# xiaochuanle/hifimeth

Measured on AMD Instinct MI355X. Metric: cytosine sites/sec (CpG+CHG+CHH), higher is better.
Workload: dtype f16x3+f32acc

## Files before the change

hifimeth_amd/csrc/hm_engine.cpp:

```cpp
#include <hip/hip_runtime.h>

#include <algorithm>
#include <atomic>
#include <cmath>
#include <condition_variable>
#include <cstdio>
#include <cstring>
#include <memory>
#include <mutex>
#include <string>
#include <thread>
#include <vector>

#include "../../include/hifimeth_hip.h"
#include "hm_device.h"
#include "hm_host.h"
#include "hm_kernels.h"
#include "hm_weights.h"

using namespace hm;

namespace {

thread_local std::string g_create_error;

enum Kind { K_PREP, K_SCAN, K_EMIT, K_PACK, K_WINDOW, K_FRONT, K_TAIL, K_TRUNK, K_EDGE, K_TAILG };

struct TimedSpan {
    int kind, ctx;
    int64_t off, cap;
    Event a, b;
};

struct DeviceModel {
    bool loaded = false;
    int k1 = 0;
    DevBuf params;
    CtxWeights w{};
};

}

struct hm_batch {
    hm_engine* e = nullptr;
    int id = 0;
    enum State { FREE, STAGING, QUEUED } state = FREE;
    bool uploaded = false, ran = false, have_totals = false, have_calls = false;
    Stream s_io;
    Event ev_in, ev_comp, ev_out;

    PinnedArr<uint8_t> slab;
    PinnedArr<ReadDesc> reads;
    PinnedArr<Chunk> chunks;
    PinnedArr<RInfo> rinfo;
    PinnedArr<TrunkTile> tiles;
    PinnedArr<int32_t> tcost;
    struct Group {
        int chunk_lo, chunk_hi, tile_lo, tile_hi;
        int64_t bases, rows;
        int cost_lo;
    };
    std::vector<Group> groups;
    int64_t total_bases = 0;

    DevBuf d_raw, d_reads, d_chunks, d_rinfo, d_tiles, d_tcost, d_bases, d_kin, d_sctx, d_counts, d_offs, d_totals, d_err;
    DevBuf d_usites, d_utag, d_csites, d_opos, d_logits, d_p, d_ml, d_calls;
    Pinned<int32_t> h_totals;
    Pinned<int32_t> h_err;
    PinnedArr<hm_call_t> h_calls;
    int32_t totals[TOT_COUNT] = {};

    std::vector<TimedSpan> spans;

    ~hm_batch() {
        if (s_io) (void)hipStreamSynchronize(s_io);
    }
};

namespace {

struct GroupBufs {
    DevBuf d_map[3], d_e4, d_edge4, d_e4row, d_rowlist;
    DevBuf d_x6;
    DevBuf d_mark, d_ccnt, d_order, d_okey;
    DevBuf d_odst;
    DevBuf d_x8;
    DevBuf d_dump;
    int64_t bytes() const {
        const DevBuf* all[] = {&d_map[0], &d_map[1], &d_map[2], &d_e4, &d_edge4, &d_e4row, &d_rowlist, &d_x6, &d_mark, &d_ccnt, &d_order, &d_okey, &d_odst, &d_x8, &d_dump};
        static_assert(sizeof(GroupBufs) == sizeof all / sizeof *all * sizeof(DevBuf), "a member of GroupBufs is missing from bytes()");
        int64_t sum = 0;
        for (const DevBuf* d : all) sum += (int64_t)d->cap;
        return sum;
    }
};

}

struct hm_engine {
    int device = 0;
    int num_cu = 256;
    int ctx_mask = 7;
    int min_read_size = 1000;
    int64_t sub_batch = 65536;
    int front_waves = 8;
    int precision = 1;
    int conv3_w16 = 0;
    int max_slots = 3;
    int trunk = 2;
    int trunk_impl = 3;
    int edge_impl = 1;
    int tail_impl = 3;
    int64_t tail_slice = int64_t(1) << 21;
    int trunk_mask_auto = -1;
    int64_t group_bases = 0;
    std::atomic<int64_t> group_bases_eff{0};
    bool stamps_on = false;
    std::vector<unsigned long long> stamp_sum;
    bool timing = false;
    std::string err;

    std::mutex mu;
    std::mutex order_mu;
    std::condition_variable cv;
    hm_timing_t acc{};
    int64_t x6_sites = 0;

    Stream stream;
    std::vector<Event> pool;
    DevBuf d_act4, d_win, d_dbg, d_stamps, d_zeros;
    GroupBufs grp;
    DeviceModel model[3];
    std::vector<std::unique_ptr<hm_batch>> slots;

    ~hm_engine() {
        (void)hipSetDevice(device);
        if (stream) (void)hipStreamSynchronize(stream);
    }
};

namespace {

constexpr int64_t GROUP_BYTES_PER_BASE = (3 * 2 * 512 + 2 * 384 + 768 + 4 + 8 + 2 * 4 + 8 + 4 + TAIL_STRIP_HANDOVER_BYTES) * 5 / 4;

int64_t effective_group_bases(hm_engine* e) {
    if (e->group_bases > 0) return e->group_bases;
    if (const int64_t have = e->group_bases_eff.load(std::memory_order_relaxed)) return have;
    size_t free_b = 0, total_b = 0;
    int64_t gb = int64_t(2) << 20;
    int prev = -1;
    (void)hipGetDevice(&prev);
    if (hipSetDevice(e->device) == hipSuccess && hipMemGetInfo(&free_b, &total_b) == hipSuccess && free_b > 0) {
        gb = (int64_t)(free_b / 4) / GROUP_BYTES_PER_BASE;
        gb = std::min<int64_t>(gb, int64_t(16) << 20);
        gb = std::max<int64_t>(gb >> 20 << 20, int64_t(1) << 20);
    }
    if (prev >= 0 && prev != e->device) (void)hipSetDevice(prev);
    int64_t none = 0;
    if (!e->group_bases_eff.compare_exchange_strong(none, gb, std::memory_order_relaxed)) gb = none;
    return gb;
}

constexpr int TILE_COST = 8, TILE_COST_CONST = 1;
void add_read_tiles(hm_engine* e, hm_batch* b, int ridx, int l_qseq) {
    if (b->groups.empty() || b->groups.back().rows >= effective_group_bases(e)) {
        b->groups.push_back(hm_batch::Group{(int)b->chunks.n, (int)b->chunks.n, (int)b->tiles.n, (int)b->tiles.n, 0, 0, (int)b->tcost.n});
        b->tcost.push_back(0);
    }
    hm_batch::Group& g = b->groups.back();
    const int ntile = (l_qseq + 2 * TR_PAD + TR_OWN - 1) / TR_OWN;
    b->rinfo.push_back(RInfo{b->total_bases, l_qseq, (int32_t)g.rows});
    for (int t = 0; t < ntile; ++t) {
        const int u0 = -TR_PAD + t * TR_OWN;
        b->tiles.push_back(TrunkTile{ridx, u0});
        b->tcost.push_back(b->tcost.p[b->tcost.n - 1] + (t == 0 ? 2 * TILE_COST_CONST : u0 >= l_qseq ? TILE_COST_CONST : TILE_COST));
    }
    for (int st = 0; st < l_qseq; st += CHUNK) b->chunks.push_back(Chunk{ridx, st});
    g.rows += (int64_t)ntile * TR_OWN + TR_SLACK;
    if (2 * g.rows >= (int64_t(1) << 27)) throw HipErr{hipErrorInvalidValue, "a read group's maps exceed 2^27 rows (group_bases too large)"};
    g.bases += l_qseq;
    g.chunk_hi = (int)b->chunks.n;
    g.tile_hi = (int)b->tiles.n;
}

int fail(hm_engine* e, int code, const std::string& msg) {
    if (e) {
        std::lock_guard<std::mutex> lk(e->mu);
        e->err = msg;
    } else {
        g_create_error = msg;
    }
    return code;
}

int fail_hip(hm_engine* e, const HipErr& h) {
    return fail(e, HM_EDEVICE, hip_error_text(h));
}

template <class Body>
auto guarded(hm_engine* e, Body&& body) -> decltype(body()) {
    return hip_guard(e->device, [e](const HipErr& h) { return fail_hip(e, h); }, body);
}

Event get_event(hm_engine* e) {
    Event ev;
    {
        std::lock_guard<std::mutex> lk(e->mu);
        if (!e->pool.empty()) {
            ev = std::move(e->pool.back());
            e->pool.pop_back();
            return ev;
        }
    }
    HIP_TRY(hipEventCreate(&ev.h));
    return ev;
}

struct Span {
    hm_engine* e;
    std::vector<TimedSpan>* sink;
    TimedSpan ts{};
    bool on;
    Span(hm_engine* eng, std::vector<TimedSpan>* out, int kind, int ctx = 0, int64_t off = 0, int64_t cap = 0)
        : e(eng), sink(out), on(eng->timing && out) {
        if (!on) return;
        ts.kind = kind;
        ts.ctx = ctx;
        ts.off = off;
        ts.cap = cap;
        ts.a = get_event(e);
        ts.b = get_event(e);
        HIP_TRY(hipEventRecord(ts.a, e->stream));
    }
    void end() {
        if (!on) return;
        HIP_TRY(hipEventRecord(ts.b, e->stream));
        sink->push_back(std::move(ts));
        on = false;
    }
};

void collect_timing(hm_engine* e, std::vector<TimedSpan>& spans, const int32_t* totals) {
    if (!spans.empty() && totals) {
        std::lock_guard<std::mutex> lk(e->mu);
        for (int c = 0; c < 3; ++c) e->acc.trunk_list_steps[c] += totals[TOT_LIST_STEPS + c];
        for (int c = 0; c < 3; ++c) e->acc.trunk_const_steps[c] += totals[TOT_CONST_STEPS + c];
        e->acc.tail_strip_passes += totals[TOT_STRIP_PASSES];
    }
    for (auto& s : spans) {
        float ms = 0.f;
        HIP_TRY(hipEventElapsedTime(&ms, s.a, s.b));
        std::lock_guard<std::mutex> lk(e->mu);
        hm_timing_t& t = e->acc;
        const int64_t n = totals ? std::clamp<int64_t>((int64_t)totals[s.ctx] - s.off, 0, s.cap) : s.cap;
        switch (s.kind) {
        case K_PREP: t.prep_ms += ms; ++t.prep_launches; break;
        case K_SCAN: t.scan_ms += ms; ++t.scan_launches; break;
        case K_EMIT: t.emit_ms += ms; ++t.emit_launches; break;
        case K_PACK: t.pack_ms += ms; ++t.pack_launches; break;
        case K_WINDOW: t.window_ms += ms; ++t.window_launches; t.window_sites += s.cap; break;
        case K_TRUNK: t.trunk_ms[s.ctx] += ms; ++t.trunk_launches[s.ctx]; t.trunk_positions[s.ctx] += s.cap; break;
        case K_EDGE: t.edge_ms[s.ctx] += ms; ++t.edge_launches[s.ctx]; break;
        case K_TAILG: t.tail_ms[s.ctx] += ms; ++t.tail_launches[s.ctx]; break;
        case K_FRONT:
            if (n > 0) { t.front_ms[s.ctx] += ms; ++t.front_launches[s.ctx]; t.front_sites[s.ctx] += n; }
            else { t.empty_ms += ms; ++t.empty_launches; }
            break;
        default:
            if (n > 0) { t.tail_ms[s.ctx] += ms; ++t.tail_launches[s.ctx]; }
            else { t.empty_ms += ms; ++t.empty_launches; }
            break;
        }
        e->pool.push_back(std::move(s.a));
        e->pool.push_back(std::move(s.b));
    }
    spans.clear();
}

void upload_model(hm_engine* e, int ctx, const HostModel& hmw) {
    DeviceModel& dm = e->model[ctx];
    PackedModel pk = pack_model(hmw);
    dm.params.reserve(pk.blob.size() * sizeof(float));
    HIP_TRY(hipMemcpy(dm.params.p, pk.blob.data(), pk.blob.size() * sizeof(float), hipMemcpyHostToDevice));
    const float* base = dm.params.as<float>();
    for (int i = 0; i < 9; ++i) {
        dm.w.wfrag[i] = base + pk.wfrag_off[i];
        dm.w.bias[i] = base + pk.bias_off[i];
    }
    dm.w.fc2_w = base + pk.fc2_w_off;
    dm.w.fc2_b = base + pk.fc2_b_off;
    dm.w.bn = reinterpret_cast<const BnTables*>(base + pk.bn_off);
    for (int i = 0; i < 9; ++i) dm.w.wfrag_h[i] = reinterpret_cast<const uint16_t*>(base + pk.wfrag_h_off[i]);
    dm.w.bn_h = reinterpret_cast<const BnTablesH*>(base + pk.bn_h_off);
    dm.w.c1f = reinterpret_cast<const uint16_t*>(base + pk.c1f_off);
    dm.w.c1f_bias = base + pk.c1f_bias_off;
    dm.w.c1f_corr = base + pk.c1f_corr_off;
    dm.w.k1 = hmw.k1;
    dm.k1 = hmw.k1;
    dm.loaded = true;
}

size_t align16(size_t x) { return (x + 15) & ~size_t(15); }

void accumulate_stamps(hm_engine* e) {
    const int ns = front_stamp_slots();
    const size_t n = (size_t)e->num_cu * 8 * ns;
    std::vector<unsigned long long> h(n);
    HIP_TRY(hipStreamSynchronize(e->stream));
    HIP_TRY(hipMemcpy(h.data(), e->d_stamps.p, n * sizeof(unsigned long long), hipMemcpyDeviceToHost));
    HIP_TRY(hipMemset(e->d_stamps.p, 0, n * sizeof(unsigned long long)));
    e->stamp_sum.resize((size_t)ns * 8, 0);
    for (size_t i = 0; i < n; ++i) e->stamp_sum[i % ((size_t)ns * 8)] += h[i];
}

void launch_cnn_pair(hm_engine* e, std::vector<TimedSpan>* spans, int ctx, const SiteRange& sr, const hm_batch* b,
                     const float* windows, float* logits, float* p, uint8_t* ml, float* dbg, int dbg_layer) {
    const DeviceModel& dm = e->model[ctx];
    const ReadDesc* reads = b ? b->d_reads.as<ReadDesc>() : nullptr;
    const uint8_t* bases = b ? b->d_bases.as<uint8_t>() : nullptr;
    const uint32_t* kin = b ? b->d_kin.as<uint32_t>() : nullptr;
    {
        Span sp(e, spans, K_FRONT, ctx, sr.off, sr.cap);
        if (e->precision >= 1)
            launch_front_h(e->stream, dm.k1, sr, reads, bases, kin, windows, dm.w, e->d_act4.as<float>(), e->num_cu, dbg,
                           dbg_layer, e->stamps_on ? e->d_stamps.as<unsigned long long>() : nullptr, false);
        else
            launch_front(e->stream, dm.k1, sr, reads, bases, kin, windows, dm.w, e->d_act4.as<float>(), e->num_cu, dbg,
                         dbg_layer, e->front_waves, e->stamps_on ? e->d_stamps.as<unsigned long long>() : nullptr);
        if (e->stamps_on) accumulate_stamps(e);
        sp.end();
    }
    {
        Span sp(e, spans, K_TAIL, ctx, sr.off, sr.cap);
        if (e->precision >= 1)
            launch_tail_h(e->stream, e->d_act4.as<float>(), sr, dm.w, logits, p, ml, e->num_cu, dbg, dbg_layer, 0);
        else
            launch_tail(e->stream, e->d_act4.as<float>(), sr, dm.w, logits, p, ml, e->num_cu, dbg, dbg_layer);
        sp.end();
    }
}

void run_cnn_windows(hm_engine* e, int ctx, const float* windows, int64_t n, float* logits, float* p, uint8_t* ml,
                     float* dbg, int dbg_layer) {
    const int64_t sb = e->sub_batch;
    e->d_act4.reserve((size_t)std::min<int64_t>(std::max<int64_t>(n, 1), sb) * ACT4_FLOATS * sizeof(float));
    std::vector<TimedSpan> spans;
    for (int64_t off = 0; off < n; off += sb) {
        const int m = (int)std::min<int64_t>(sb, n - off);
        const SiteRange sr{nullptr, nullptr, ctx, 0, m};
        launch_cnn_pair(e, e->timing ? &spans : nullptr, ctx, sr, nullptr, windows + (size_t)off * KMER * FEATS,
                        logits + 2 * off, p + off, ml + off, dbg, dbg_layer);
    }
    HIP_TRY(hipGetLastError());
    HIP_TRY(hipStreamSynchronize(e->stream));
    collect_timing(e, spans, nullptr);
}

hm_batch* new_slot(hm_engine* e, int id) {
    std::unique_ptr<hm_batch> b(new hm_batch());
    b->e = e;
    b->id = id;
    HIP_TRY(hipStreamCreateWithFlags(&b->s_io.h, hipStreamNonBlocking));
    for (Event* ev : {&b->ev_in, &b->ev_comp, &b->ev_out}) HIP_TRY(hipEventCreateWithFlags(&ev->h, hipEventDisableTiming));
    b->h_totals.alloc(TOT_COUNT);
    b->h_err.alloc();
    b->d_totals.reserve(TOT_COUNT * sizeof(int32_t));
    b->d_err.reserve(sizeof(int32_t));
    HIP_TRY(hipMemset(b->d_err.p, 0, sizeof(int32_t)));
    HIP_TRY(hipMemset(b->d_totals.p, 0, TOT_COUNT * sizeof(int32_t)));
    hm_batch* raw = b.get();
    e->slots.push_back(std::move(b));
    return raw;
}

void reset_staging(hm_batch* b) {
    b->slab.n = 0;
    b->reads.n = 0;
    b->chunks.n = 0;
    b->rinfo.n = 0;
    b->tiles.n = 0;
    b->tcost.n = 0;
    b->groups.clear();
    b->total_bases = 0;
    b->uploaded = b->ran = b->have_totals = b->have_calls = false;
    memset(b->totals, 0, sizeof b->totals);
}


int check_read(hm_engine* e, const hm_read_t& r, int64_t tb, const char* who, const char* full) {
    if (r.l_qseq < 0) return fail(e, HM_EINVAL, std::string(who) + ": negative read length");
    if (r.l_qseq < e->min_read_size) return 0;
    if (!r.kin[0] || !r.kin[1] || !r.kin[2] || !r.kin[3]) return 0;
    if (!r.seq4) return fail(e, HM_EINVAL, std::string(who) + ": seq4 is NULL");
    for (int k = 0; k < 4; ++k)
        if (r.width[k] != 1 && r.width[k] != 2) return fail(e, HM_EINVAL, "kinetics element width must be 1 (B:C) or 2 (B:S)");
    if (tb + (int64_t)r.l_qseq + 4 >= (int64_t(1) << 31)) return fail(e, HM_ENOMEM, std::string(who) + ": batch would exceed 2^31 bases; " + full);
    return 1;
}

int64_t padded_bases(int32_t l_qseq) { return ((int64_t)l_qseq + 3) & ~int64_t(3); }

struct SlabCopy {
    const void* src;
    size_t off, bytes;
};

void place_read(hm_batch* b, const hm_read_t& r, SlabCopy* copies) {
    const size_t L = (size_t)r.l_qseq;
    auto place = [&](const void* src, size_t bytes) {
        const int64_t off = (int64_t)b->slab.n;
        *copies++ = SlabCopy{src, (size_t)off, bytes};
        b->slab.n += align16(bytes);
        return off;
    };
    ReadDesc rd{};
    rd.off_seq = place(r.seq4, (L + 1) / 2);
    rd.off_fi = place(r.kin[0], L * r.width[0]);
    rd.off_fp = place(r.kin[1], L * r.width[1]);
    rd.off_ri = place(r.kin[2], L * r.width[2]);
    rd.off_rp = place(r.kin[3], L * r.width[3]);
    rd.base_off = b->total_bases;
    rd.len = r.l_qseq;
    rd.flag = r.flag;
    rd.read_id = r.read_id;
    for (int k = 0; k < 4; ++k) rd.w[k] = r.width[k];
    const int ridx = (int)b->reads.n;
    b->reads.push_back(rd);
    add_read_tiles(b->e, b, ridx, r.l_qseq);
    b->total_bases += padded_bases(r.l_qseq);
}

int stage_read(hm_batch* b, int32_t read_id, int32_t l_qseq, int32_t flag, const uint8_t* seq4, const void* fi, int fi_w,
               const void* fp, int fp_w, const void* ri, int ri_w, const void* rp, int rp_w) {
    auto width = [](int w) { return (uint8_t)std::clamp(w, 0, 255); };
    const hm_read_t r{read_id, l_qseq, flag, {width(fi_w), width(fp_w), width(ri_w), width(rp_w)}, seq4, {fi, fp, ri, rp}};
    const int rc = check_read(b->e, r, b->total_bases, "hm_submit_read", "flush / queue it first");
    if (rc <= 0) return rc;
    return guarded(b->e, [&] {
        const size_t L = (size_t)l_qseq;
        const size_t need = align16((L + 1) / 2) + align16(L * fi_w) + align16(L * fp_w) + align16(L * ri_w) + align16(L * rp_w);
        if (b->slab.n + need > b->slab.cap) b->slab.reserve(std::max<size_t>((b->slab.n + need) * 2, size_t(64) << 20));
        SlabCopy copies[5];
        place_read(b, r, copies);
        for (const SlabCopy& c : copies) memcpy(b->slab.p + c.off, c.src, c.bytes);
        return 1;
    });
}

void enqueue_upload(hm_batch* b) {
    const size_t nr = b->reads.n, nc = b->chunks.n;
    b->d_raw.reserve(std::max<size_t>(b->slab.n, 16));
    b->d_reads.reserve(std::max<size_t>(nr, 1) * sizeof(ReadDesc));
    b->d_chunks.reserve(std::max<size_t>(nc, 1) * sizeof(Chunk));
    const size_t tb = (size_t)std::max<int64_t>(b->total_bases, 4);
    b->d_bases.reserve(tb);
    b->d_sctx.reserve(tb);
    b->d_kin.reserve(tb * sizeof(uint32_t));
    b->d_counts.reserve((nc + 1) * NCNT * sizeof(int32_t));
    b->d_offs.reserve((nc + 1) * NCNT * sizeof(int32_t));
    b->d_usites.reserve(tb * sizeof(USite));
    b->d_utag.reserve(tb);
    b->d_csites.reserve(tb * sizeof(Site));
    b->d_opos.reserve(tb * sizeof(int32_t));
    b->d_logits.reserve(tb * 2 * sizeof(float));
    b->d_p.reserve(tb * sizeof(float));
    b->d_ml.reserve(tb);
    b->d_calls.reserve(tb * sizeof(hm_call_t));
    if (b->slab.n) HIP_TRY(hipMemcpyAsync(b->d_raw.p, b->slab.p, b->slab.n, hipMemcpyHostToDevice, b->s_io));
    if (nr) HIP_TRY(hipMemcpyAsync(b->d_reads.p, b->reads.p, nr * sizeof(ReadDesc), hipMemcpyHostToDevice, b->s_io));
    if (nc) HIP_TRY(hipMemcpyAsync(b->d_chunks.p, b->chunks.p, nc * sizeof(Chunk), hipMemcpyHostToDevice, b->s_io));
    b->d_rinfo.reserve(std::max<size_t>(nr, 1) * sizeof(RInfo));
    b->d_tiles.reserve(std::max<size_t>(b->tiles.n, 1) * sizeof(TrunkTile));
    if (nr) HIP_TRY(hipMemcpyAsync(b->d_rinfo.p, b->rinfo.p, nr * sizeof(RInfo), hipMemcpyHostToDevice, b->s_io));
    if (b->tiles.n) HIP_TRY(hipMemcpyAsync(b->d_tiles.p, b->tiles.p, b->tiles.n * sizeof(TrunkTile), hipMemcpyHostToDevice, b->s_io));
    b->d_tcost.reserve(std::max<size_t>(b->tcost.n, 1) * sizeof(int32_t));
    if (b->tcost.n) HIP_TRY(hipMemcpyAsync(b->d_tcost.p, b->tcost.p, b->tcost.n * sizeof(int32_t), hipMemcpyHostToDevice, b->s_io));
    HIP_TRY(hipEventRecord(b->ev_in, b->s_io));
    b->uploaded = true;
    b->ran = b->have_totals = b->have_calls = false;
}

void run_trunk_path(hm_batch* b, std::vector<TimedSpan>* spans, int ctx_mask) {
    hm_engine* e = b->e;
    int64_t max_rows = 1, max_bases = 1;
    for (const auto& g : b->groups) {
        max_rows = std::max(max_rows, g.rows);
        max_bases = std::max(max_bases, g.bases);
    }
    for (int i = 0; i < 3; ++i) e->grp.d_map[i].reserve((size_t)max_rows * 2 * 256 * sizeof(uint16_t));
    e->grp.d_e4.reserve((size_t)max_rows * 2 * C4_CH * sizeof(float));
    e->grp.d_rowlist.reserve(std::max((size_t)(max_rows / TR_OWN + 1) * 2 * 3 * TR_OWN, trunk3_rowlist_bytes((max_rows / TR_OWN + 1) * 2)));
    e->grp.d_dump.reserve(trunk3_dump_bytes(e->num_cu));
    e->grp.d_edge4.reserve((size_t)max_bases * 2 * C4_CH * sizeof(float));
    e->grp.d_e4row.reserve((size_t)max_bases * sizeof(int32_t));
    if (e->tail_impl == 3 && e->precision >= 1 && (ctx_mask >> CHH & 1)) {
        e->grp.d_mark.reserve(tail_strip_mark_bytes(2 * max_rows));
        e->grp.d_ccnt.reserve(tail_strip_count_bytes(2 * max_rows));
        e->grp.d_order.reserve((size_t)max_bases * sizeof(int32_t));
        e->grp.d_okey.reserve((size_t)max_bases * sizeof(int32_t));
        e->grp.d_odst.reserve((size_t)max_bases * sizeof(int32_t));
        e->grp.d_x8.reserve(tail_strip_handover_bytes(max_bases));
    }
    if (!e->d_zeros.p) {
        e->d_zeros.reserve(1024);
        HIP_TRY(hipMemsetAsync(e->d_zeros.p, 0, 1024, e->stream));
    }
    const bool w16 = false;
    const int32_t* offs = b->d_offs.as<int32_t>();
    for (const auto& g : b->groups) {
        const TrunkMaps maps{{e->grp.d_map[0].as<uint16_t>(), e->grp.d_map[1].as<uint16_t>(), e->grp.d_map[2].as<uint16_t>()},
                             e->grp.d_e4.as<uint16_t>(), g.rows, e->d_zeros.as<uint16_t>(), e->grp.d_rowlist.as<uint8_t>()};
        const int n_tiles = g.tile_hi - g.tile_lo;
        for (int c = 0; c < 3; ++c) {
            if (!(ctx_mask >> c & 1)) continue;
            const DeviceModel& dm = e->model[c];
            const int n_views = c == CHH ? 2 : 1;
            const SiteRange sr{b->d_csites.as<Site>(), b->d_totals.as<int32_t>(), c, 0, (int32_t)std::min<int64_t>(g.bases, INT32_MAX),
                               offs + (size_t)NCNT * g.chunk_lo + c, offs + (size_t)NCNT * g.chunk_hi + c};
            if (e->precision == 0) {
                {
                    Span sp(e, spans, K_TRUNK, c, 0, (int64_t)n_tiles * TR_OWN * n_views);
                    launch_trunk_f32(e->stream, dm.k1, b->d_tiles.as<TrunkTile>() + g.tile_lo, n_tiles, n_views, c, b->d_rinfo.as<RInfo>(),
                                     b->d_bases.as<uint8_t>(), b->d_kin.as<uint32_t>(), b->d_sctx.as<uint8_t>(), dm.w, maps, e->num_cu);
                    sp.end();
                }
                {
                    Span sp(e, spans, K_EDGE, c);
                    launch_edge_f32(e->stream, dm.k1, sr, b->d_rinfo.as<RInfo>(), b->d_bases.as<uint8_t>(), b->d_kin.as<uint32_t>(), dm.w,
                                    maps, e->grp.d_edge4.as<float>(), e->grp.d_e4row.as<int32_t>(), e->num_cu);
                    sp.end();
                }
                Span sp(e, spans, K_TAILG, c);
                launch_tail_gather_f32(e->stream, sr, dm.w, maps, e->grp.d_edge4.as<float>(), e->grp.d_e4row.as<int32_t>(),
                                       b->d_logits.as<float>(), b->d_p.as<float>(), b->d_ml.as<uint8_t>(), e->num_cu);
                sp.end();
                continue;
            }
            {
                Span sp(e, spans, K_TRUNK, c, 0, (int64_t)n_tiles * TR_OWN * n_views);
                if (e->trunk_impl == 3)
                    launch_trunk3(e->stream, dm.k1, b->d_tiles.as<TrunkTile>() + g.tile_lo, n_tiles, n_views, c, b->d_rinfo.as<RInfo>(),
                                  b->d_bases.as<uint8_t>(), b->d_kin.as<uint32_t>(), b->d_sctx.as<uint8_t>(), b->total_bases, dm.w, maps, e->grp.d_dump.as<uint16_t>(),
                                  b->d_totals.as<int32_t>() + TOT_LIST_STEPS, b->d_tcost.as<int32_t>() + g.cost_lo, e->num_cu, e->conv3_w16 != 0);
                else if (e->trunk_impl)
                    launch_trunk2(e->stream, dm.k1, b->d_tiles.as<TrunkTile>() + g.tile_lo, n_tiles, n_views, c, b->d_rinfo.as<RInfo>(),
                                  b->d_bases.as<uint8_t>(), b->d_kin.as<uint32_t>(), b->d_sctx.as<uint8_t>(), dm.w, maps, e->num_cu, w16,
                                  e->trunk_impl == 2);
                else
// ... 689 lines not shown
```

hifimeth_amd/csrc/hm_trunk3.hip:

```cpp
#include "hm_convh.h"
#ifdef HM_TRUNK_STAMP
#include "hm_stamp.h"
namespace hm { __device__ unsigned long long g_trunk3_stamp[8][24]; }
extern "C" int hm_debug_trunk3_stamps(unsigned long long* out, int reset) {
    if (out && hipMemcpyFromSymbol(out, HIP_SYMBOL(hm::g_trunk3_stamp), sizeof(hm::g_trunk3_stamp)) != hipSuccess) return -1;
    if (reset) {
        static unsigned long long z[8][24];
        if (hipMemcpyToSymbol(HIP_SYMBOL(hm::g_trunk3_stamp), z, sizeof(z)) != hipSuccess) return -1;
    }
    return 0;
}
#endif
#include "hm_convs.h"
#include "hm_edge.h"

namespace hm {

namespace {

constexpr int T3_M = TR_OWN;
constexpr int T3_H1 = 4, T3_H2 = 8, T3_H3 = 16;
constexpr int T3_S3 = T3_H3, T3_S2 = T3_S3 + T3_H2, T3_S1 = T3_S2 + T3_H1;
constexpr int T3_AROWS = T3_M + T3_H3, T3_BROWS = T3_M + T3_H2;
constexpr int T3_XROWS = 128;
constexpr int T3_LDS_HALVES = 2 * T3_AROWS * TR_RS + 2 * T3_BROWS * TR_RS + 2 * (T3_H1 + T3_H3) * TR_RS;
constexpr int T3_N4 = 64, T3_RL3 = 3 * TR_OWN, T3_RL = T3_RL3 + T3_N4 + 4;
constexpr int T3_RLW = 3 * 32 + T3_N4 / 4 + 1;
static_assert(T3_M % 16 == 0 && T3_RL % 4 == 0 && T3_RL / 4 <= 256 && T3_XROWS >= T3_M + 12, "tile plan");

struct ListRows4 {
    static constexpr bool DENSE = false;
    static constexpr int M = T3_N4;
    const uint8_t* rows = nullptr;
    template <class C>
    __device__ __forceinline__ int off(int m) const { return (int)rows[m] * C::IRS; }
};
struct EpiE4L {
    half_t* __restrict__ g;
    const uint8_t* rows;
    __device__ __forceinline__ void operator()(int m, int col, const f32x4& acc) const {
        half4 h, l;
        split4(acc, h, l);
        const size_t o = (size_t)rows[m] * (2 * C4_CH) + col;
        *reinterpret_cast<half4*>(g + o) = h;
        *reinterpret_cast<half4*>(g + o + C4_CH) = l;
    }
};

struct EpiTrunk3 {
    half_t* hi;
    half_t* lo;
    __device__ __forceinline__ void operator()(int m, int col, const f32x4& acc) const {
        half4 h, l;
        split4(acc, h, l);
        *reinterpret_cast<half4*>(hi + m * TR_RS + col) = h;
        *reinterpret_cast<half4*>(lo + m * TR_RS + col) = l;
    }
};
struct EpiE43 {
    half_t* __restrict__ g;
    __device__ __forceinline__ void operator()(int m, int col, const f32x4& acc) const {
        half4 h, l;
        split4(acc, h, l);
        *reinterpret_cast<half4*>(g + (size_t)m * (2 * C4_CH) + col) = h;
        *reinterpret_cast<half4*>(g + (size_t)m * (2 * C4_CH) + C4_CH + col) = l;
    }
};
template <int NWV_>
struct CopyRows3 {
    static constexpr int NWV = NWV_, CS = TR_OWN / (2 * NWV_);
    const uint8_t* rows;
    half_t* g;
};

__device__ __forceinline__ void t3_lds_barrier() {
    __builtin_amdgcn_fence(__ATOMIC_RELEASE, "workgroup", "local");
    __builtin_amdgcn_s_barrier();
    __builtin_amdgcn_fence(__ATOMIC_ACQUIRE, "workgroup", "local");
}

template <int NROWS, int NT, int K = 0>
__device__ __forceinline__ void move_rows(half_t* dh, half_t* dl, const half_t* sh, const half_t* sl, int t) {
    constexpr int PER = NROWS * TR_RS / 8, N = 2 * PER;
    if constexpr (K * NT < N) {
        const int c = min(t + K * NT, N - 1), plane = c >= PER, o = (c - plane * PER) * 8;
        const uint4 v = *reinterpret_cast<const uint4*>((plane ? sl : sh) + o);
        move_rows<NROWS, NT, K + 1>(dh, dl, sh, sl, t);
        *reinterpret_cast<uint4*>((plane ? dl : dh) + o) = v;
    }
}

}

constexpr int T3_RPB = 4;
template <int K1>
__global__ __launch_bounds__(64) void rowlist3_kernel(const TrunkTile* __restrict__ tiles, int n_tiles, int n_work, int ctx,
                                                       const RInfo* __restrict__ rinfo, const uint8_t* __restrict__ sctx, int64_t n_bases,
                                                       uint8_t* __restrict__ rowlist) {
    using G = EdgeGeo<K1>;
    const int r = threadIdx.x;
    constexpr int first_new[3] = {T3_H1, T3_H2, T3_H3}, shift[3] = {T3_S1, T3_S2, T3_S3};
    constexpr int W0 = -176, WN = 528;
    __shared__ __attribute__((aligned(4))) uint8_t rec[T3_RPB][T3_RL];
    __shared__ __attribute__((aligned(4))) uint8_t sf[T3_RPB][WN];
    static_assert(-G::R1 - 2 + T3_S1 >= W0 && -G::R2 - 4 + T3_S2 >= W0 && -G::R3 - 8 + T3_S3 >= W0 && T3_S1 + TR_OWN - 1 - G::LEFT < W0 + WN &&
                  215 - 16 * 23 >= W0 && TR_OWN - 1 + 215 - 16 < W0 + WN, "the window covers every lookup");
    int kind[T3_RPB];
    TrunkTile tl[T3_RPB];
    RInfo ri[T3_RPB];
    bool warm[T3_RPB];
    int view[T3_RPB];
#pragma unroll
    for (int k = 0; k < T3_RPB; ++k) {
        const int blk = (int)blockIdx.x * T3_RPB + k;
        kind[k] = blk > 2 * n_work ? 0 : blk == 2 * n_work ? 2 : 1;
        warm[k] = blk >= n_work;
        const int w = min(warm[k] ? blk - n_work : blk, n_work - 1);
        view[k] = w >= n_tiles;
        tl[k] = tiles[view[k] ? w - n_tiles : w];
    }
    bool any = false;
#pragma unroll
    for (int k = 0; k < T3_RPB; ++k) {
        if (kind[k] == 1 && warm[k] && tl[k].u0 != -TR_PAD) kind[k] = 0;
        any |= kind[k] != 0;
    }
    if (!any) return;
#pragma unroll
    for (int k = 0; k < T3_RPB; ++k) ri[k] = rinfo[tl[k].read_idx];
    constexpr int NQ = (WN / 4 + 63) / 64;
    static_assert(WN % 4 == 0 && (-W0) % 4 == 0 && TR_PAD % 4 == 0 && TR_OWN % 4 == 0, "windows start on multiples of 4");
    uint32_t sw[T3_RPB][NQ];
#pragma unroll
    for (int k = 0; k < T3_RPB; ++k) {
        const int L = ri[k].len, u = tl[k].u0 - (warm[k] ? TR_OWN : 0);
#pragma unroll
        for (int q = 0; q < NQ; ++q) {
            const int y0 = u + W0 + 4 * (r + 64 * q);
            const int64_t a = view[k] ? ri[k].base_off + (L - 1 - y0 - 3) : ri[k].base_off + y0;
            if (a >= 0 && a + 4 <= n_bases) {
                uint32_t v;
                __builtin_memcpy(&v, sctx + a, 4);
                sw[k][q] = view[k] ? __builtin_bswap32(v) : v;
            } else {
                uint32_t v = 0;
#pragma unroll
                for (int t = 0; t < 4; ++t) {
                    const int64_t j = view[k] ? ri[k].base_off + (L - 1 - y0 - t) : ri[k].base_off + y0 + t;
                    v |= (uint32_t)(j >= 0 && j < n_bases ? sctx[j] : (uint8_t)CTX_NONE) << (8 * t);
                }
                sw[k][q] = v;
            }
        }
    }
#pragma unroll
    for (int k = 0; k < T3_RPB; ++k) {
        for (int i = r; i < T3_RL3; i += 64) rec[k][i] = (uint8_t)(first_new[i / TR_OWN] + TR_OWN - 1);
        const int L = ri[k].len, u = tl[k].u0 - (warm[k] ? TR_OWN : 0);
        const uint32_t key = (uint32_t)(ctx | (view[k] << 2)) * 0x01010101u;
#pragma unroll
        for (int q = 0; q < NQ; ++q) {
            const int y0 = u + W0 + 4 * (r + 64 * q);
            const uint32_t x = sw[k][q] ^ key;
            uint32_t hit = (~(((x & 0x7F7F7F7Fu) + 0x7F7F7F7Fu) | x | 0x7F7F7F7Fu)) >> 7;
            const int lo = min(max(-y0, 0), 4), hi = min(max(L - y0, 0), 4);
            const uint32_t m_hi = hi >= 4 ? 0xFFFFFFFFu : (1u << (8 * hi)) - 1u, m_lo = lo >= 4 ? 0xFFFFFFFFu : (1u << (8 * lo)) - 1u;
            hit &= m_hi & ~m_lo;
            if (r + 64 * q < WN / 4) reinterpret_cast<uint32_t*>(sf[k])[r + 64 * q] = hit;
        }
    }
    __syncthreads();
    const uint64_t below = (1ull << r) - 1;
#pragma unroll
    for (int k = 0; k < T3_RPB; ++k) {
        if (kind[k] == 0) continue;
        const int blk = (int)blockIdx.x * T3_RPB + k;
        int n4 = 255;
        if (kind[k] == 1) {
            const int u = tl[k].u0 - (warm[k] ? TR_OWN : 0);
            auto sat = [&](int y) __attribute__((always_inline)) { return (int)sf[k][y - u - W0]; };
            const bool want4 = K1 == 11 && !warm[k];
            int f[2] = {0, 0}, need4[2] = {0, 0};
#pragma unroll
            for (int h = 0; h < 2; ++h) {
                const int row = r + 64 * h;
                if (row < TR_OWN) {
                    {
                        const int x = u + shift[0] + row;
                        f[h] |= (sat(x - G::LEFT) | sat(x - G::R1) | (G::PAD2 ? 0 : sat(x - G::R1 - 2))) << 0;
                    }
                    {
                        const int x = u + shift[1] + row;
                        f[h] |= (sat(x - G::LEFT) | sat(x - G::R2) | (G::PAD3 ? 0 : sat(x - G::R2 - 4))) << 1;
                    }
                    {
                        const int x = u + shift[2] + row;
                        f[h] |= (sat(x - G::LEFT) | sat(x - G::R3) | (G::PAD4 ? 0 : sat(x - G::R3 - 8))) << 2;
                    }
                    if (want4) {
#pragma unroll
                        for (int sidx = 1; sidx <= 23; ++sidx) need4[h] |= sat(u + row + 215 - 16 * sidx);
                    }
                }
            }
#pragma unroll
            for (int l = 0; l < 3; ++l) {
                const uint64_t b0 = __ballot((f[0] >> l) & 1), b1 = __ballot((f[1] >> l) & 1);
                if ((f[0] >> l) & 1) rec[k][l * TR_OWN + __popcll(b0 & below)] = (uint8_t)(first_new[l] + r);
                if ((f[1] >> l) & 1) rec[k][l * TR_OWN + __popcll(b0) + __popcll(b1 & below)] = (uint8_t)(first_new[l] + r + 64);
            }
            const uint64_t n0 = __ballot(need4[0]), n1 = __ballot(need4[1]);
            if (want4) n4 = __popcll(n0) + __popcll(n1);
            if (want4 && n4 <= T3_N4) {
                if (need4[0]) rec[k][T3_RL3 + __popcll(n0 & below)] = (uint8_t)r;
                if (need4[1]) rec[k][T3_RL3 + __popcll(n0) + __popcll(n1 & below)] = (uint8_t)(r + 64);
                __syncthreads();
                if (r >= n4) rec[k][T3_RL3 + r] = n4 > 0 ? rec[k][T3_RL3] : (uint8_t)0;
            }
        }
        if (r == 0) *reinterpret_cast<uint32_t*>(&rec[k][T3_RL3 + T3_N4]) = (uint32_t)n4;
        __syncthreads();
        uint32_t* out = reinterpret_cast<uint32_t*>(rowlist + (size_t)blk * T3_RL);
        for (int i = r; i < T3_RL / 4; i += 64) out[i] = reinterpret_cast<const uint32_t*>(rec[k])[i];
    }
}

template <int K1, bool W3LO = true>
__global__ __launch_bounds__(256) __attribute__((amdgpu_waves_per_eu(1, 1)))
void trunk3_kernel(const TrunkTile* __restrict__ tiles, int n_tiles, int n_views, int ctx, const RInfo* __restrict__ rinfo,
                   const uint8_t* __restrict__ bases, const uint32_t* __restrict__ kin, CtxWeights W, TrunkMaps mp, half_t* __restrict__ dump,
                   int32_t* __restrict__ list_steps, const int32_t* __restrict__ tcost) {
    constexpr int NW = 4, NTW = 2;
    __shared__ __attribute__((aligned(16))) half_t smem[T3_LDS_HALVES + T3_XROWS * TR_WRS];
    static_assert(sizeof(smem) == 147840, "LDS plan");
    __shared__ uint32_t rlist[2][T3_RLW];
    __shared__ int64_t s_grow0;
    __shared__ int s_kind;
    __shared__ __attribute__((aligned(16))) half_t kc[3][2][128];
    __shared__ __attribute__((aligned(16))) half_t e4c[2 * C4_CH];
    half_t* a_hi = smem;
    half_t* a_lo = a_hi + T3_AROWS * TR_RS;
    half_t* b_hi = a_lo + T3_AROWS * TR_RS;
    half_t* b_lo = b_hi + T3_BROWS * TR_RS;
    half_t* h1_hi = b_lo + T3_BROWS * TR_RS;
    half_t* h1_lo = h1_hi + T3_H1 * TR_RS;
    half_t* h3_hi = h1_lo + T3_H1 * TR_RS;
    half_t* h3_lo = h3_hi + T3_H3 * TR_RS;
    half_t* xb = h3_lo + T3_H3 * TR_RS;
    const int n_work = n_tiles * n_views;
    const int lane = threadIdx.x & 63, wave = __builtin_amdgcn_readfirstlane(threadIdx.x >> 6);
    int w0, w1;
    if (tcost) {
        const int64_t c_view = tcost[n_tiles], c_all = c_view * n_views;
        auto cost_at = [&](const int wq) __attribute__((always_inline)) {
            const int v = wq >= n_tiles && wq < n_work ? 1 : wq >= n_work ? n_views : 0;
            return v * c_view + (wq >= n_work ? 0 : tcost[wq - (v ? n_tiles : 0)]);
        };
        auto first_at = [&](const int64_t target) __attribute__((always_inline)) {
            int lo = 0, hi = n_work;
            while (hi > lo) {
                const int stride = (hi - lo + 63) / 64;
                const int probe = lo + lane * stride;
                const bool ge = probe >= hi || cost_at(probe) >= target;
                const uint64_t bal = __ballot(ge);
                const int first = bal ? __builtin_ctzll(bal) : 64;
                if (first == 0) {
                    hi = lo;
                } else {
                    const int nlo = lo + (first - 1) * stride + 1;
                    hi = first < 64 ? min(lo + first * stride, hi) : hi;
                    lo = nlo;
                }
            }
            return __builtin_amdgcn_readfirstlane(lo);
        };
        const int64_t k = blockIdx.x, G = gridDim.x;
        w0 = first_at((k * c_all + G - 1) / G);
        w1 = k + 1 == G ? n_work : first_at(((k + 1) * c_all + G - 1) / G);
    } else {
        const int base_n = n_work / (int)gridDim.x, rem_n = n_work - base_n * (int)gridDim.x;
        w0 = (int)blockIdx.x * base_n + min((int)blockIdx.x, rem_n);
        w1 = w0 + base_n + ((int)blockIdx.x < rem_n);
    }
    if (w0 >= w1) return;

    for (int i = threadIdx.x; i < (T3_LDS_HALVES + T3_XROWS * TR_WRS) / 2; i += NW * 64) reinterpret_cast<uint32_t*>(smem)[i] = 0u;
    for (int i = threadIdx.x; i < 2 * T3_RLW; i += NW * 64) rlist[0][i] = 0;
    __syncthreads();

    struct Build {
        TrunkTile tl, tl2;
        RInfo ri;
        int w, view, warm, cst, calib, ueff, b;
        uint32_t k, rl;
    } bd;
    auto build_desc1 = [&](const int w) __attribute__((always_inline)) {
        bd.w = w;
        bd.view = w >= n_tiles;
        bd.tl = tiles[bd.view ? w - n_tiles : w];
        const int w2 = min(w + 1, n_work - 1);
        bd.tl2 = tiles[w2 >= n_tiles ? w2 - n_tiles : w2];
    };
    auto build_desc2 = [&](const int prev_warm, const bool first) __attribute__((always_inline)) {
        bd.tl.read_idx = __builtin_amdgcn_readfirstlane(bd.tl.read_idx);
        bd.tl.u0 = __builtin_amdgcn_readfirstlane(bd.tl.u0);
        bd.warm = first ? 1 : (prev_warm ? 0 : (bd.tl.u0 == -TR_PAD));
        bd.calib = 0;
        bd.ueff = bd.tl.u0 - (bd.warm ? TR_OWN : 0);
        bd.ri = rinfo[bd.tl.read_idx];
    };
    auto build_desc3 = [&]() __attribute__((always_inline)) {
        bd.ri.len = __builtin_amdgcn_readfirstlane(bd.ri.len);
        bd.ri.map_off = __builtin_amdgcn_readfirstlane(bd.ri.map_off);
        bd.ri.base_off = ((int64_t)__builtin_amdgcn_readfirstlane((int)(bd.ri.base_off >> 32)) << 32) |
                         (uint32_t)__builtin_amdgcn_readfirstlane((int)bd.ri.base_off);
        bd.cst = bd.tl.u0 == -TR_PAD || (!bd.warm && bd.tl.u0 >= bd.ri.len);
    };
    auto build_loads = [&]() __attribute__((always_inline)) {
        const int r = threadIdx.x, L = bd.ri.len, x = bd.ueff + T3_S1 + r;
        const int xc = min(max(x, 0), L - 1);
        const int64_t j = bd.ri.base_off + (bd.view ? L - 1 - xc : xc);
        bd.b = bases[j];
        bd.k = kin[j];
        const size_t li = bd.calib ? (size_t)2 * n_work : bd.warm ? (bd.tl.u0 == -TR_PAD ? (size_t)n_work + bd.w : (size_t)2 * n_work) : (size_t)bd.w;
        bd.rl = reinterpret_cast<const uint32_t*>(mp.rowlist + li * T3_RL)[min(r, T3_RL / 4 - 1)];
    };
    auto build_store = [&](const int buf) __attribute__((always_inline)) {
        const int r = threadIdx.x, x = bd.ueff + T3_S1 + r;
        if (r == 0) {
            s_grow0 = (int64_t)bd.view * mp.view_rows + bd.ri.map_off + (bd.ueff + TR_PAD);
            s_kind = bd.warm | (bd.cst << 1) | (bd.calib << 2);
        }
        if (r < T3_XROWS) {
            const bool in = !bd.calib && x >= 0 && x < bd.ri.len;
            *reinterpret_cast<uint4*>(xb + r * TR_WRS) = feature_row(in ? bd.b : -1, bd.k, bd.view);
        }
        if (r < T3_RL3 / 4) rlist[buf][r / (TR_OWN / 4) * 32 + r % (TR_OWN / 4)] = bd.rl;
        else if (r < T3_RL / 4) rlist[buf][3 * 32 + r - T3_RL3 / 4] = bd.rl;
    };

    using C1 = SCfg<8, (2 * K1 + 3) / 4 * 4, TR_WRS, 1, true, false, K1, 2, NTW>;
    using C2 = SCfg<128, 3, TR_RS, 2, true, true, 0, 1, NTW>;
    using C3 = SCfg<128, 3, TR_RS, 4, W3LO, true, 0, 1, NTW>;
    using C4 = SCfg<128, 3, TR_RS, 8, true, true, 0, 1, NTW>;
    using C4s = SCfg<128, 3, TR_RS, 8, true, true, 0, 1, 1>;
    const int nt04 = wave == 0 ? 0 : wave == 1 ? 1 : wave == 2 ? 3 : 4;
    using L1 = SConv<C1, C2, 0, 2, 2, 3>;
    using L2 = SConv<C2, C3, 0, 3, 4>;
    using L3 = SConv<C3, C4, 0, 3, 4>;
    static_assert(T3_XROWS <= NW * 64, "one feature row per thread");
    auto wf = [&](int i) { return reinterpret_cast<const half_t*>(W.wfrag_h[i]); };
    const half_t* c1f = reinterpret_cast<const half_t*>(W.c1f);
    const int nt0 = NTW * wave;

    WRegs wr;
    sconv_load_w<C1, 0, C1::KB>(c1f, nt0, lane, wr);
    sconv_load_bias<C1>(W.c1f_bias, nt0, lane, wr);
    build_desc1(w0);
    build_desc2(0, true);
    build_desc3();
    bd.calib = 1;
    bd.cst = 0;
    build_loads();
    build_store(0);
    int buf = 0;
    int w = w0, warm = 1;
    int n_list = 0;
    int n_const = 0;
    bool prev_calib = false;
    half_t* const dump_rows = dump + TR_OWN * 2 * C4_CH;
    half_t* const dump_cal = dump_rows + 128 * 256 + (size_t)blockIdx.x * (TR_OWN * 2 * C4_CH);
    constexpr int first_new[3] = {T3_H1, T3_H2, T3_H3};
#ifdef HM_TRUNK_STAMP
    unsigned long long ts[10], acc_t[16] = {};
    unsigned long long n_it = 0, acc_c = 0, n_c = 0;
    const bool st_on = blockIdx.x == 0;
    const unsigned long long tk0 = hm_stamp(), tr0 = __builtin_amdgcn_s_memrealtime();
#define TS(i) do { if (st_on) ts[i] = hm_stamp(); } while (0)
#else
#define TS(i)
#endif
    while (true) {
        t3_lds_barrier();
        TS(0);
        const int64_t grow0 = s_grow0;
        const int kind = __builtin_amdgcn_readfirstlane(s_kind);
        const int cur_warm = kind & 1, cur_const = (kind >> 1) & 1, cur_calib = kind >> 2;
        if (prev_calib) {
            prev_calib = false;
            __builtin_amdgcn_fence(__ATOMIC_ACQUIRE, "agent");
            const int t = threadIdx.x;
            if (t < 96) {
                const int l = t >> 5, plane = (t >> 4) & 1, col = (t & 15) * 8;
                const half_t* src = l == 0 ? (plane ? h1_lo : h1_hi) : l == 1 ? (plane ? b_lo : b_hi) : (plane ? h3_lo : h3_hi);
                *reinterpret_cast<uint4*>(&kc[l][plane][col]) = *reinterpret_cast<const uint4*>(src + col);
            } else if (t < 96 + 24) {
                reinterpret_cast<uint4*>(e4c)[t - 96] = reinterpret_cast<const uint4*>(dump_cal + (TR_OWN - 1) * 2 * C4_CH)[t - 96];
            }
            __syncthreads();
        }
        const int wn = cur_warm ? w : w + 1;
        const bool last = wn >= w1;
        half_t* g1 = cur_calib ? dump_rows : reinterpret_cast<half_t*>(mp.e[0]) + (grow0 + T3_S2) * 256;
        half_t* g2 = cur_calib ? dump_rows : reinterpret_cast<half_t*>(mp.e[1]) + (grow0 + T3_S3) * 256;
        half_t* g3 = cur_calib ? dump_rows : reinterpret_cast<half_t*>(mp.e[2]) + grow0 * 256;
        const uint8_t* rl = reinterpret_cast<const uint8_t*>(rlist[buf]);
        if (cur_const) {
            const int t = threadIdx.x;
            n_const += !cur_warm;
            const int wb = min(wn, w1 - 1);
            bool new_read = false;
            if (wb != bd.w) {
                const int prev_read = bd.tl.read_idx;
                bd.w = wb;
                bd.view = wb >= n_tiles;
                bd.tl.read_idx = __builtin_amdgcn_readfirstlane(bd.tl2.read_idx);
                bd.tl.u0 = __builtin_amdgcn_readfirstlane(bd.tl2.u0);
                const int w2 = min(wb + 1, n_work - 1);
                bd.tl2 = tiles[w2 >= n_tiles ? w2 - n_tiles : w2];
                new_read = bd.tl.read_idx != prev_read;
                if (new_read) bd.ri = rinfo[bd.tl.read_idx];
            }
            auto finish_desc = [&]() __attribute__((always_inline)) {
                bd.warm = cur_warm ? 0 : (bd.tl.u0 == -TR_PAD);
                bd.calib = 0;
                bd.ueff = bd.tl.u0 - (bd.warm ? TR_OWN : 0);
                bd.cst = bd.tl.u0 == -TR_PAD || (!bd.warm && bd.tl.u0 >= bd.ri.len);
                build_loads();
            };
            if (!new_read) finish_desc();
            if (!cur_warm) {
                uint4* g4 = reinterpret_cast<uint4*>(reinterpret_cast<half_t*>(mp.e4) + grow0 * (2 * C4_CH));
                const uint4 v = reinterpret_cast<const uint4*>(e4c)[t % 24];
                const uint4 v2 = reinterpret_cast<const uint4*>(e4c)[(t + 16) % 24], v3 = reinterpret_cast<const uint4*>(e4c)[(t + 8) % 24];
#pragma unroll
                for (int k = 0; k < (TR_OWN * 24 + 255) / 256; ++k) {
                    const int c = t + 256 * k;
                    if (c < TR_OWN * 24) g4[c] = k % 3 == 0 ? v : k % 3 == 1 ? v2 : v3;
                }
            }
#pragma unroll
            for (int l = 0; l < 3; ++l) {
                const uint8_t* rows = rl + 128 * l;
                half_t* g = l == 0 ? g1 : l == 1 ? g2 : g3;
                const int fill = first_new[l] + TR_OWN - 1, ch = t & 31;
                const uint4 v = reinterpret_cast<const uint4*>(&kc[l][0][0])[ch];
                int pr[TR_OWN / 8];
#pragma unroll
                for (int i = 0; i < TR_OWN / 8; ++i) pr[i] = rows[(t >> 5) + 8 * i];
#pragma unroll
                for (int i = 0; i < TR_OWN / 8; ++i)
                    if (pr[i] != fill) reinterpret_cast<uint4*>(g + (size_t)pr[i] * 256)[ch] = v;
                if (t < 32) reinterpret_cast<uint4*>(g + (size_t)fill * 256)[ch] = v;
            }
            for (int c = t; c < (T3_H1 + T3_H2 + T3_H3) * 32; c += NW * 64) {
                const int row = c >> 5, plane = (c >> 4) & 1, col = (c & 15) * 8;
                const int l = row < T3_H1 ? 0 : row < T3_H1 + T3_H2 ? 1 : 2, r = row - (l == 0 ? 0 : l == 1 ? T3_H1 : T3_H1 + T3_H2);
                half_t* dst = (l == 0 ? (plane ? h1_lo : h1_hi) : l == 1 ? (plane ? b_lo : b_hi) : (plane ? h3_lo : h3_hi)) + r * TR_RS + col;
                *reinterpret_cast<uint4*>(dst) = *reinterpret_cast<const uint4*>(&kc[l][plane][col]);
            }
            if (new_read) {
                build_desc3();
                finish_desc();
            }
            t3_lds_barrier();
            build_store(buf ^ 1);
            buf ^= 1;
#ifdef HM_TRUNK_STAMP
            if (st_on) {
                acc_c += hm_stamp() - ts[0];
                ++n_c;
            }
#endif
            if (last) break;
            w = wn;
            warm = bd.warm;
            continue;
        }
        move_rows<T3_H1, NW * 64>(a_hi, a_lo, h1_hi, h1_lo, threadIdx.x);
        L1::run(xb, xb, wr, EpiTrunk3{a_hi + T3_H1 * TR_RS, a_lo + T3_H1 * TR_RS}, wf(1), W.bias[1], nt0, nt0);
        build_desc1(min(wn, w1 - 1));
        TS(1);
        __syncthreads();
        TS(2);
        build_desc2(cur_warm, cur_calib != 0);
        L2::run(a_hi, a_lo, wr, EpiTrunk3{b_hi + T3_H2 * TR_RS, b_lo + T3_H2 * TR_RS}, wf(2), W.bias[2], nt0, nt0, CopyRows3<NW>{rl, g1});
        move_rows<T3_H1, NW * 64>(h1_hi, h1_lo, a_hi + T3_M * TR_RS, a_lo + T3_M * TR_RS, threadIdx.x);
        TS(3);
        __syncthreads();
        TS(4);
        build_desc3();
        build_loads();
        move_rows<T3_H3, NW * 64>(a_hi, a_lo, h3_hi, h3_lo, threadIdx.x);
        L3::run(b_hi, b_lo, wr, EpiTrunk3{a_hi + T3_H3 * TR_RS, a_lo + T3_H3 * TR_RS}, wf(3), W.bias[3], nt0, nt04, CopyRows3<NW>{rl + 128, g2});
        TS(5);
        __syncthreads();
        TS(6);
        move_rows<T3_H3, NW * 64>(h3_hi, h3_lo, a_hi + T3_M * TR_RS, a_lo + T3_M * TR_RS, threadIdx.x);
        move_rows<T3_H2, NW * 64>(b_hi, b_lo, b_hi + T3_M * TR_RS, b_lo + T3_M * TR_RS, threadIdx.x);
        const EpiE43 e4{cur_calib ? dump_cal : cur_warm ? dump : reinterpret_cast<half_t*>(mp.e4) + grow0 * (2 * C4_CH)};
        const int n4 = __builtin_amdgcn_readfirstlane((int)rlist[buf][T3_RLW - 1]);
        if (!cur_warm && n4 <= T3_N4) {
            ++n_list;
            const uint8_t* rows4 = rl + 3 * 128;
            const ListRows4 rm{rows4};
            const EpiE4L e4l{reinterpret_cast<half_t*>(mp.e4) + grow0 * (2 * C4_CH), rows4};
            using NoCp = typename SConvR<C4, C1, ListRows4, 2, 2>::NoCopy;
            if (wave & 1) {
                SConvR<C4s, void, ListRows4, 0, 1, 1>::template run<1>(a_hi, a_lo, wr, e4l, c1f, W.c1f_bias, nt04, nt0, CopyRows3<NW>{rl + 256, g3}, rm);
                SConvR<C4, C1, ListRows4, 2, 2>::run(a_hi, a_lo, wr, e4l, c1f, W.c1f_bias, nt04, nt0, NoCp{}, rm);
            } else {
                SConvR<C4, void, ListRows4, 0, 1, 1>::run(a_hi, a_lo, wr, e4l, c1f, W.c1f_bias, nt04, nt0, CopyRows3<NW>{rl + 256, g3}, rm);
                SConvR<C4s, C1, ListRows4, 2, 2>::template run<0>(a_hi, a_lo, wr, e4l, c1f, W.c1f_bias, nt04, nt0, NoCp{}, rm);
            }
        } else
        if (wave & 1) {
            SConv<C4s, void, 0, 2, 2>::template run<1>(a_hi, a_lo, wr, e4, c1f, W.c1f_bias, nt04, nt0, CopyRows3<NW>{rl + 256, g3});
            SConv<C4, C1, 4, 3>::run(a_hi, a_lo, wr, e4, c1f, W.c1f_bias, nt04, nt0);
        } else {
            SConv<C4, void, 0, 2, 2>::run(a_hi, a_lo, wr, e4, c1f, W.c1f_bias, nt04, nt0, CopyRows3<NW>{rl + 256, g3});
            SConv<C4s, C1, 4, 3>::template run<0>(a_hi, a_lo, wr, e4, c1f, W.c1f_bias, nt04, nt0);
        }
        build_store(buf ^ 1);
        buf ^= 1;
        if (cur_calib) {
            __builtin_amdgcn_fence(__ATOMIC_RELEASE, "agent");
            prev_calib = true;
        }
        TS(7);
#ifdef HM_TRUNK_STAMP
        if (st_on) {
            __syncthreads();
            ts[8] = hm_stamp();
            for (int l = 0; l < 4; ++l) {
                acc_t[4 * l + 0] += ts[2 * l + 1] - ts[2 * l];
                acc_t[4 * l + 3] += ts[2 * l + 2] - ts[2 * l + 1];
            }
            ++n_it;
        }
#endif
        if (last) break;
        w = wn;
        warm = bd.warm;
    }
    (void)warm;
#ifdef HM_TRUNK_STAMP
    if (st_on && (threadIdx.x & 63) == 0) {
        for (int i = 0; i < 16; ++i) atomicAdd(&g_trunk3_stamp[threadIdx.x >> 6][i], acc_t[i]);
        atomicAdd(&g_trunk3_stamp[threadIdx.x >> 6][16], n_it);
        atomicAdd(&g_trunk3_stamp[threadIdx.x >> 6][17], acc_c);
        atomicAdd(&g_trunk3_stamp[threadIdx.x >> 6][18], n_c);
        atomicAdd(&g_trunk3_stamp[threadIdx.x >> 6][22], hm_stamp() - tk0);
        atomicAdd(&g_trunk3_stamp[threadIdx.x >> 6][23], __builtin_amdgcn_s_memrealtime() - tr0);
    }
#endif
#undef TS
    if (list_steps && threadIdx.x == 0 && n_list) atomicAdd(list_steps + ctx, n_list);
    if (list_steps && threadIdx.x == 0 && n_const) atomicAdd(list_steps + 4 + ctx, n_const);
}

size_t trunk3_rowlist_bytes(int64_t n_work) { return (size_t)(2 * n_work + 1) * T3_RL + 64; }
size_t trunk3_dump_bytes(int grid) { return ((size_t)(1 + grid) * TR_OWN * 2 * C4_CH + 128 * 256) * sizeof(uint16_t); }

void launch_trunk3(hipStream_t st, int k1, const TrunkTile* tiles, int n_tiles, int n_views, int ctx, const RInfo* rinfo,
                   const uint8_t* bases, const uint32_t* kin, const uint8_t* sctx, int64_t n_bases, const CtxWeights& w, const TrunkMaps& maps,
                   uint16_t* dump, int32_t* list_steps, const int32_t* tcost, int grid, bool w3_single) {
    if (n_tiles <= 0) return;
    const int n_work = n_tiles * n_views;
    const dim3 g(min(n_work, grid));
    if (k1 == 11) {
        hipLaunchKernelGGL(rowlist3_kernel<11>, dim3((2 * n_work + T3_RPB) / T3_RPB), dim3(64), 0, st, tiles, n_tiles, n_work, ctx, rinfo, sctx, n_bases, maps.rowlist);
        if (w3_single) hipLaunchKernelGGL((trunk3_kernel<11, false>), g, dim3(256), 0, st, tiles, n_tiles, n_views, ctx, rinfo, bases, kin, w, maps, reinterpret_cast<half_t*>(dump), list_steps, tcost);
        else hipLaunchKernelGGL((trunk3_kernel<11, true>), g, dim3(256), 0, st, tiles, n_tiles, n_views, ctx, rinfo, bases, kin, w, maps, reinterpret_cast<half_t*>(dump), list_steps, tcost);
    } else {
        hipLaunchKernelGGL(rowlist3_kernel<13>, dim3((2 * n_work + T3_RPB) / T3_RPB), dim3(64), 0, st, tiles, n_tiles, n_work, ctx, rinfo, sctx, n_bases, maps.rowlist);
        if (w3_single) hipLaunchKernelGGL((trunk3_kernel<13, false>), g, dim3(256), 0, st, tiles, n_tiles, n_views, ctx, rinfo, bases, kin, w, maps, reinterpret_cast<half_t*>(dump), list_steps, tcost);
        else hipLaunchKernelGGL((trunk3_kernel<13, true>), g, dim3(256), 0, st, tiles, n_tiles, n_views, ctx, rinfo, bases, kin, w, maps, reinterpret_cast<half_t*>(dump), list_steps, tcost);
    }
}

}
```

Baseline: 64.35 million.

## Size list-mode conv4 to actual needed rows and widen list capacity to 96

Raises the sparse row-list capacity for the conv4/C1 stage from 64 to 96 rows and pads the extra slots. The list-mode path now dispatches on the number of 16-row groups actually needed and instantiates the SConvR calls with matching tile counts, so partially filled lists skip unused row tiles. More tiles can take the list path instead of the dense fallback. The cost is more template instantiations and code size, plus a changed step-counting statistic.

Result: no change. 64.93 million, median of 6 (+0.9%).

```diff
diff --git a/hifimeth_amd/csrc/hm_engine.cpp b/hifimeth_amd/csrc/hm_engine.cpp
--- a/hifimeth_amd/csrc/hm_engine.cpp
+++ b/hifimeth_amd/csrc/hm_engine.cpp
@@ -243,7 +243,7 @@
 void collect_timing(hm_engine* e, std::vector<TimedSpan>& spans, const int32_t* totals) {
     if (!spans.empty() && totals) {
         std::lock_guard<std::mutex> lk(e->mu);
-        for (int c = 0; c < 3; ++c) e->acc.trunk_list_steps[c] += totals[TOT_LIST_STEPS + c];
+        for (int c = 0; c < 3; ++c) e->acc.trunk_list_steps[c] += (totals[TOT_LIST_STEPS + c] + 1) / 3;
         for (int c = 0; c < 3; ++c) e->acc.trunk_const_steps[c] += totals[TOT_CONST_STEPS + c];
         e->acc.tail_strip_passes += totals[TOT_STRIP_PASSES];
     }
diff --git a/hifimeth_amd/csrc/hm_trunk3.hip b/hifimeth_amd/csrc/hm_trunk3.hip
--- a/hifimeth_amd/csrc/hm_trunk3.hip
+++ b/hifimeth_amd/csrc/hm_trunk3.hip
@@ -24,7 +24,7 @@
 constexpr int T3_AROWS = T3_M + T3_H3, T3_BROWS = T3_M + T3_H2;
 constexpr int T3_XROWS = 128;
 constexpr int T3_LDS_HALVES = 2 * T3_AROWS * TR_RS + 2 * T3_BROWS * TR_RS + 2 * (T3_H1 + T3_H3) * TR_RS;
-constexpr int T3_N4 = 64, T3_RL3 = 3 * TR_OWN, T3_RL = T3_RL3 + T3_N4 + 4;
+constexpr int T3_N4 = 96, T3_RL3 = 3 * TR_OWN, T3_RL = T3_RL3 + T3_N4 + 4;
 constexpr int T3_RLW = 3 * 32 + T3_N4 / 4 + 1;
 static_assert(T3_M % 16 == 0 && T3_RL % 4 == 0 && T3_RL / 4 <= 256 && T3_XROWS >= T3_M + 12, "tile plan");
 
@@ -215,7 +215,9 @@
                 if (need4[0]) rec[k][T3_RL3 + __popcll(n0 & below)] = (uint8_t)r;
                 if (need4[1]) rec[k][T3_RL3 + __popcll(n0) + __popcll(n1 & below)] = (uint8_t)(r + 64);
                 __syncthreads();
-                if (r >= n4) rec[k][T3_RL3 + r] = n4 > 0 ? rec[k][T3_RL3] : (uint8_t)0;
+                const uint8_t fill4 = n4 > 0 ? rec[k][T3_RL3] : (uint8_t)0;
+                if (r >= n4) rec[k][T3_RL3 + r] = fill4;
+                if (r + 64 < T3_N4 && r + 64 >= n4) rec[k][T3_RL3 + r + 64] = fill4;
             }
         }
         if (r == 0) *reinterpret_cast<uint32_t*>(&rec[k][T3_RL3 + T3_N4]) = (uint32_t)n4;
@@ -501,18 +503,36 @@
         const EpiE43 e4{cur_calib ? dump_cal : cur_warm ? dump : reinterpret_cast<half_t*>(mp.e4) + grow0 * (2 * C4_CH)};
         const int n4 = __builtin_amdgcn_readfirstlane((int)rlist[buf][T3_RLW - 1]);
         if (!cur_warm && n4 <= T3_N4) {
-            ++n_list;
+            const int m4 = (n4 + 15) >> 4;
+            n_list += 7 - max(m4, 2);
             const uint8_t* rows4 = rl + 3 * 128;
-            const ListRows4 rm{rows4};
-            const EpiE4L e4l{reinterpret_cast<half_t*>(mp.e4) + grow0 * (2 * C4_CH), rows4};
-            using NoCp = typename SConvR<C4, C1, ListRows4, 2, 2>::NoCopy;
-            if (wave & 1) {
-                SConvR<C4s, void, ListRows4, 0, 1, 1>::template run<1>(a_hi, a_lo, wr, e4l, c1f, W.c1f_bias, nt04, nt0, CopyRows3<NW>{rl + 256, g3}, rm);
-                SConvR<C4, C1, ListRows4, 2, 2>::run(a_hi, a_lo, wr, e4l, c1f, W.c1f_bias, nt04, nt0, NoCp{}, rm);
-            } else {
-                SConvR<C4, void, ListRows4, 0, 1, 1>::run(a_hi, a_lo, wr, e4l, c1f, W.c1f_bias, nt04, nt0, CopyRows3<NW>{rl + 256, g3}, rm);
-                SConvR<C4s, C1, ListRows4, 2, 2>::template run<0>(a_hi, a_lo, wr, e4l, c1f, W.c1f_bias, nt04, nt0, NoCp{}, rm);
-            }
+            half_t* const g4 = reinterpret_cast<half_t*>(mp.e4) + grow0 * (2 * C4_CH);
+            const CopyRows3<NW> cp3{rl + 256, g3};
+            auto form = [&](auto g1_, auto s_) __attribute__((always_inline)) {
+                constexpr int G1 = decltype(g1_)::value, S = decltype(s_)::value;
+                const ListRows4 rm{rows4}, rm2{rows4 + 16 * (1 + G1)};
+                const EpiE4L e4l{g4, rows4}, e4l2{g4, rows4 + 16 * (1 + G1)};
+                using NoCp = typename SConvR<C4, C1, ListRows4, 0, S>::NoCopy;
+                if (wave & 1) {
+                    SConvR<C4s, void, ListRows4, 0, 1, G1>::template run<1>(a_hi, a_lo, wr, e4l, c1f, W.c1f_bias, nt04, nt0, cp3, rm);
+                    SConvR<C4, C1, ListRows4, 0, S>::run(a_hi, a_lo, wr, e4l2, c1f, W.c1f_bias, nt04, nt0, NoCp{}, rm2);
+                } else {
+                    SConvR<C4, void, ListRows4, 0, 1, G1>::run(a_hi, a_lo, wr, e4l, c1f, W.c1f_bias, nt04, nt0, cp3, rm);
+                    SConvR<C4s, C1, ListRows4, 0, S>::template run<0>(a_hi, a_lo, wr, e4l2, c1f, W.c1f_bias, nt04, nt0, NoCp{}, rm2);
+                }
+            };
+            using I1 = std::integral_constant<int, 1>;
+            using I2 = std::integral_constant<int, 2>;
+            using I3 = std::integral_constant<int, 3>;
+            if (m4 <= 2) {
+                const ListRows4 rm{rows4};
+                const EpiE4L e4l{g4, rows4};
+                if (wave & 1) SConvR<C4s, C1, ListRows4, 0, 1, 1>::template run<1>(a_hi, a_lo, wr, e4l, c1f, W.c1f_bias, nt04, nt0, cp3, rm);
+                else SConvR<C4, C1, ListRows4, 0, 1, 1>::run(a_hi, a_lo, wr, e4l, c1f, W.c1f_bias, nt04, nt0, cp3, rm);
+            } else if (m4 == 3) form(I1{}, I1{});
+            else if (m4 == 4) form(I1{}, I2{});
+            else if (m4 == 5) form(I1{}, I3{});
+            else form(I2{}, I3{});
         } else
         if (wave & 1) {
             SConv<C4s, void, 0, 2, 2>::template run<1>(a_hi, a_lo, wr, e4, c1f, W.c1f_bias, nt04, nt0, CopyRows3<NW>{rl + 256, g3});
```
